# leo27945875/Python_Stable_3D_Truss_Analysis

Measured on AMD Instinct MI355X. Metric: truss solves/sec (batched Solve), higher is better.
Workload: dtype f64; 1 GPU; bar-942_input_0 x 4096 independent copies per GPU (nJ 244, nM 942, n_free 696); batch_per_gpu=4096, parallelism=batch-sharded x1, no collective

## Files before the change

### python_stable_3d_truss_analysis_amd/csrc/order.hip

```cpp
#include "trs_common.h"
#include "../../include/trs_solver.h"
#include <type_traits>

namespace {

#ifndef TRS_ORDER_THREADS
#define TRS_ORDER_THREADS 256
#endif
constexpr int NT = TRS_ORDER_THREADS;
constexpr int NWAVE = NT / 64;
static_assert(NT == 128 || NT == 256 || NT == 512, "two, four or eight waves");
constexpr int ID_BITS = 13;
constexpr int PERMANENT = 0x40000000;
constexpr unsigned long long NO_COST = ~0ull;
constexpr int RCM_BELOW = 128;

struct OrdLds {
    size_t nfr, deg, start, fill, lvl, ppos, queue, nextq, order, ids, frank, bins, adj, adjU, keys,
        cand, best, newidx, c01, cmin, ctrl, red, total;
    int nch_max, n4;
};
__host__ __device__ inline size_t ord_up(size_t v) { return (v + 15) / 16 * 16; }
__host__ __device__ inline OrdLds ord_layout(int nJ_max, int nM_max) {
    OrdLds l;
    const size_t n = (size_t)nJ_max, e = 2 * (size_t)(nM_max < 1 ? 1 : nM_max);
    l.nch_max = 3 * nJ_max / 16 + 8;
    size_t p = 0;
    auto take = [&](size_t bytes) { const size_t at = p; p += ord_up(bytes); return at; };
    l.nfr = take(n);
    l.deg = take(4 * n);
    l.start = take(4 * (n + 1));
    l.fill = take(4 * n);
    l.lvl = take(4 * n);
    l.ppos = take(4 * n);
    l.queue = take(2 * n);
    l.nextq = take(2 * n);
    l.order = take(2 * n);
    l.ids = take(2 * n);
    l.frank = take(2 * (n + 1));
    l.bins = take(2 * 3 * n);
    l.adj = take(2 * (e + 4));
    const size_t shared_at = p;
    l.adjU = take(4 * (e + 4));
    const size_t lists_end = p;
    p = shared_at;
    l.n4 = (nJ_max + 3) / 4 * 4;
    l.keys = take(4 * (size_t)l.n4 * NWAVE);
    l.cand = take(2 * n * NWAVE);
    l.best = take(2 * n * NWAVE);
    l.newidx = take(2 * n * NWAVE);
    l.c01 = take(2 * n * NWAVE);
    p = p > lists_end ? p : lists_end;
    l.cmin = take(4 * (size_t)l.nch_max * NWAVE);
    l.ctrl = take(4 * 32);
    l.red = take(8 * 64);
    l.total = p;
    return l;
}

__device__ __forceinline__ int wave_incl_scan(int v, int lane) {
#pragma unroll
    for (int off = 1; off < 64; off <<= 1) {
        const int up = __shfl_up(v, off);
        if (lane >= off) v += up;
    }
    return v;
}

template <typename T, typename F>
__device__ __forceinline__ T block_reduce(T v, T* red, F op) {
#pragma unroll
    for (int off = 32; off > 0; off >>= 1) v = op(v, __shfl_xor(v, off));
    __syncthreads();
    if ((threadIdx.x & 63) == 0) red[threadIdx.x >> 6] = v;
    __syncthreads();
    T r = red[0];
#pragma unroll
    for (int w = 1; w < NWAVE; ++w) r = op(r, red[w]);
    return r;
}

#ifdef TRS_ORDER_STAMPS
__device__ unsigned long long g_ord_stamps[16];
struct OrdStamp {
    unsigned long long t0;
    __device__ OrdStamp() : t0(__builtin_amdgcn_s_memtime()) {}
    __device__ void mark(int slot) {
        const unsigned long long t = __builtin_amdgcn_s_memtime();
        if ((threadIdx.x & 63) == 0) atomicAdd(&g_ord_stamps[slot], t - t0);
        t0 = t;
    }
};
#else
struct OrdStamp {
    __device__ void mark(int) {}
};
#endif


struct Tables {
    unsigned char* nfr;
    int *deg, *start, *fill, *lvl, *ppos;
    unsigned short *queue, *nextq, *order;
    unsigned short *ids, *frank, *bins, *adj;
    unsigned* adjU;
    unsigned long long* keys;
    unsigned short *cand, *best, *newidx, *c01;
    int *cmin, *ctrl;
    unsigned long long* red;
};

template <bool SORTED>
__device__ int bfs_sweep(const Tables& t, int nj, int root, int stamp, int* last_begin) {
    const int tid = threadIdx.x;
    int* found_cnt = t.ctrl;
    if constexpr (SORTED)
        for (int j = tid; j < nj; j += NT) t.ppos[j] = 0x7fffffff;
    if (tid == 0) {
        t.queue[0] = (unsigned short)root;
        t.lvl[root] = stamp;
        found_cnt[0] = 0;
    }
    __syncthreads();
    unsigned short* found = SORTED ? t.nextq : t.queue;
    int head = 0, tail = 1, depth = 0, begin = 0, turn = 0;
    const int sub = tid & 3;
    while (head < tail) {
        begin = head;
        const int mark = stamp + depth + 1;
        int* my_cnt = found_cnt + turn;
        const int next_turn = turn == 2 ? 0 : turn + 1, slot0 = tail;
        if (tid == 0) found_cnt[next_turn] = 0;
        for (int i = head + (tid >> 2); i < tail; i += NT / 4) {
            const int v = t.queue[i];
            const int e1 = t.start[v + 1];
            for (int e = t.start[v] + sub; e < e1; e += 4) {
                const int w = t.adj[e];
                const int old = atomicMax(&t.lvl[w], mark);
                if (old < stamp) found[slot0 + atomicAdd(my_cnt, 1)] = (unsigned short)w;
                if (SORTED && (old < stamp || old == mark)) atomicMin(&t.ppos[w], i);
            }
        }
        __syncthreads();
        const int new_tail = slot0 + *my_cnt;
        if constexpr (SORTED) {
            const int m = new_tail - tail;
            if (m > 1) {
                for (int x = tid; x < m; x += NT) {
                    const int w = t.nextq[tail + x];
                    t.keys[x] = ((unsigned long long)t.ppos[w] << 40) | ((unsigned long long)t.deg[w] << 20) |
                                (unsigned long long)w;
                }
                __syncthreads();
                for (int x = tid; x < m; x += NT) {
                    const unsigned long long mine = t.keys[x];
                    int rank = 0;
                    for (int y = 0; y < m; ++y) rank += t.keys[y] < mine ? 1 : 0;
                    t.queue[tail + rank] = (unsigned short)(mine & 0xfffffu);
                }
            } else if (m == 1 && tid == 0) {
                t.queue[tail] = t.nextq[tail];
            }
            __syncthreads();
        }
        head = tail;
        tail = new_tail;
        turn = next_turn;
        ++depth;
    }
    *last_begin = begin;
    return tail;
}

template <typename Ord>
__device__ unsigned long long price_order(const Tables& t, int nf, Ord ord, unsigned short* newidx,
                                          unsigned short* c01, int* cmin, int lane, int* n_out) {
    int carry = 0;
    for (int base = 0; base < nf; base += 64) {
        const int k = base + lane;
        const int old = k < nf ? ord(k) : 0;
        const int v = k < nf ? (int)t.nfr[old] : 0;
        const int incl = wave_incl_scan(v, lane);
        const int ds = carry + incl - v;
        if (k < nf) {
            newidx[old] = (unsigned short)k;
            c01[k] = (unsigned short)(((ds >> 4) << 1) | ((((ds + v - 1) >> 4) != (ds >> 4)) ? 1 : 0));
        }
        carry += __shfl(incl, 63);
    }
    const int n = carry, nch = (n + 15) >> 4;
    for (int q = lane; q < nch; q += 64) cmin[q] = q;
    __builtin_amdgcn_wave_barrier();
    for (int k = lane; k < nf; k += 64) {
        const int old = ord(k);
        int m = k;
        const int e1 = t.start[old + 1];
        for (int e = t.start[old]; e < e1; e += 4) {
            const int w0 = t.adj[e], w1 = t.adj[e + 1], w2 = t.adj[e + 2], w3 = t.adj[e + 3];
            const int i0 = newidx[w0], i1 = e + 1 < e1 ? (int)newidx[w1] : k, i2 = e + 2 < e1 ? (int)newidx[w2] : k,
                      i3 = e + 3 < e1 ? (int)newidx[w3] : k;
            m = min(min(m, i0), min(min(i1, i2), i3));
        }
        const int col = c01[m] >> 1, mine = c01[k];
        atomicMin(&cmin[mine >> 1], col);
        if (mine & 1) atomicMin(&cmin[(mine >> 1) + 1], col);
    }
    __builtin_amdgcn_wave_barrier();
    unsigned long long cost = 0;
    int run = nch;
    for (int base = (nch - 1) / 64 * 64; base >= 0; base -= 64) {
        const int q = base + lane;
        int v = q < nch ? cmin[q] : 0x7fffffff;
#pragma unroll
        for (int off = 1; off < 64; off <<= 1) {
            const int o = __shfl_down(v, off);
            if (lane + off < 64) v = min(v, o);
        }
        v = min(v, run);
        if (q < nch) {
            const unsigned long long w = (unsigned long long)(q - v + 1);
            cost += w * (w + 12ull);
        }
        run = __shfl(v, 0);
    }
#pragma unroll
    for (int off = 32; off > 0; off >>= 1) cost += __shfl_xor(cost, off);
    __builtin_amdgcn_wave_barrier();
    *n_out = n;
    return cost;
}

template <typename Fwd>
__device__ void price_order_pair(const Tables& t, int nf, Fwd fwd, unsigned short* newidx, unsigned short* c01,
                                 int* cmin, unsigned short* c01r, int* cminr, int lane, int* n_out,
                                 unsigned long long* cost_fwd, unsigned long long* cost_rev) {
    auto pack = [](int ds, int v) { return (unsigned short)(((ds >> 4) << 1) | ((((ds + v - 1) >> 4) != (ds >> 4)) ? 1 : 0)); };
    int carry = 0;
    for (int base = 0; base < nf; base += 64) {
        const int k = base + lane;
        const int old = k < nf ? fwd(k) : 0;
        const int v = k < nf ? (int)t.nfr[old] : 0;
        const int incl = wave_incl_scan(v, lane);
        const int ds = carry + incl - v;
        if (k < nf) {
            newidx[old] = (unsigned short)k;
            c01[k] = pack(ds, v);
            c01r[k] = (unsigned short)(ds + v);
        }
        carry += __shfl(incl, 63);
    }
    const int n = carry, nch = (n + 15) >> 4;
    for (int q = lane; q < nch; q += 64) {
        cmin[q] = q;
        cminr[q] = q;
    }
    __builtin_amdgcn_wave_barrier();
    for (int k = lane; k < nf; k += 64) {
        const int end = c01r[k];
        c01r[k] = pack(n - end, (int)t.nfr[fwd(k)]);
    }
    __builtin_amdgcn_wave_barrier();
    for (int k = lane; k < nf; k += 64) {
        const int old = fwd(k);
        int lo = k, hi = k;
        const int e1 = t.start[old + 1];
        for (int e = t.start[old]; e < e1; e += 4) {
            const int w0 = t.adj[e], w1 = t.adj[e + 1], w2 = t.adj[e + 2], w3 = t.adj[e + 3];
            const int i0 = newidx[w0], i1 = e + 1 < e1 ? (int)newidx[w1] : k, i2 = e + 2 < e1 ? (int)newidx[w2] : k,
                      i3 = e + 3 < e1 ? (int)newidx[w3] : k;
            lo = min(min(lo, i0), min(min(i1, i2), i3));
            hi = max(max(hi, i0), max(max(i1, i2), i3));
        }
        const int col = c01[lo] >> 1, mine = c01[k];
        atomicMin(&cmin[mine >> 1], col);
        if (mine & 1) atomicMin(&cmin[(mine >> 1) + 1], col);
        const int colr = c01r[hi] >> 1, miner = c01r[k];
        atomicMin(&cminr[miner >> 1], colr);
        if (miner & 1) atomicMin(&cminr[(miner >> 1) + 1], colr);
    }
    __builtin_amdgcn_wave_barrier();
    unsigned long long cf = 0, cr = 0;
    int runf = nch, runr = nch;
    for (int base = (nch - 1) / 64 * 64; base >= 0; base -= 64) {
        const int q = base + lane;
        int vf = q < nch ? cmin[q] : 0x7fffffff, vr = q < nch ? cminr[q] : 0x7fffffff;
#pragma unroll
        for (int off = 1; off < 64; off <<= 1) {
            const int of = __shfl_down(vf, off), orv = __shfl_down(vr, off);
            if (lane + off < 64) {
                vf = min(vf, of);
                vr = min(vr, orv);
            }
        }
        vf = min(vf, runf);
        vr = min(vr, runr);
        if (q < nch) {
            const unsigned long long wf = (unsigned long long)(q - vf + 1), wr = (unsigned long long)(q - vr + 1);
            cf += wf * (wf + 12ull);
            cr += wr * (wr + 12ull);
        }
        runf = __shfl(vf, 0);
        runr = __shfl(vr, 0);
    }
#pragma unroll
    for (int off = 32; off > 0; off >>= 1) {
        cf += __shfl_xor(cf, off);
        cr += __shfl_xor(cr, off);
    }
    __builtin_amdgcn_wave_barrier();
    *n_out = n;
    *cost_fwd = cf;
    *cost_rev = cr;
}

__global__ __launch_bounds__(NT, 4) void trs_joint_order_kernel(
    const double* __restrict__ xyz, const void* __restrict__ conn, const unsigned char* __restrict__ cbits,
    const double* __restrict__ loads, const int* __restrict__ nJ_arr, const int* __restrict__ nM_arr,
    const int nJ_max, const int nM_max, int* __restrict__ perm_out, int* __restrict__ choice_out,
    int* __restrict__ reach_out, double* __restrict__ xyz_out, void* __restrict__ conn_out,
    unsigned char* __restrict__ cbits_out, double* __restrict__ loads_out, const int effort,
    const long long* __restrict__ rows, const int nJ_in, const int nM_in, const double* __restrict__ E_in,
    const double* __restrict__ A_in, double* __restrict__ E_out, double* __restrict__ A_out,
    int* __restrict__ nJ_out, int* __restrict__ nM_out,
    const int conn16, const unsigned char* __restrict__ tidx_in, unsigned char* __restrict__ tidx_out) {
    extern __shared__ unsigned char lds[];
    const int b = blockIdx.x, tid = threadIdx.x, lane = tid & 63;
    const int wave = __builtin_amdgcn_readfirstlane(tid >> 6);
    const size_t src = rows != nullptr ? (size_t)rows[b] : (size_t)b;
    const int nJ_src = rows != nullptr ? nJ_in : nJ_max, nM_src = rows != nullptr ? nM_in : nM_max;
    const int nj = nJ_arr[src], nm = nM_arr[src];
    const OrdLds lay = ord_layout(nJ_max, nM_max);
    Tables t;
    t.nfr = lds + lay.nfr;
    t.deg = reinterpret_cast<int*>(lds + lay.deg);
    t.start = reinterpret_cast<int*>(lds + lay.start);
    t.fill = reinterpret_cast<int*>(lds + lay.fill);
    t.lvl = reinterpret_cast<int*>(lds + lay.lvl);
    t.ppos = reinterpret_cast<int*>(lds + lay.ppos);
    t.queue = reinterpret_cast<unsigned short*>(lds + lay.queue);
    t.nextq = reinterpret_cast<unsigned short*>(lds + lay.nextq);
    t.order = reinterpret_cast<unsigned short*>(lds + lay.order);
    t.ids = reinterpret_cast<unsigned short*>(lds + lay.ids);
    t.frank = reinterpret_cast<unsigned short*>(lds + lay.frank);
    t.bins = reinterpret_cast<unsigned short*>(lds + lay.bins);
    t.adj = reinterpret_cast<unsigned short*>(lds + lay.adj);
    t.adjU = reinterpret_cast<unsigned*>(lds + lay.adjU);
    t.keys = reinterpret_cast<unsigned long long*>(lds + lay.keys);
    t.cand = reinterpret_cast<unsigned short*>(lds + lay.cand);
    t.best = reinterpret_cast<unsigned short*>(lds + lay.best);
    t.newidx = reinterpret_cast<unsigned short*>(lds + lay.newidx);
    t.c01 = reinterpret_cast<unsigned short*>(lds + lay.c01);
    t.cmin = reinterpret_cast<int*>(lds + lay.cmin);
    t.ctrl = reinterpret_cast<int*>(lds + lay.ctrl);
    t.red = reinterpret_cast<unsigned long long*>(lds + lay.red);

    const unsigned char* CB = cbits + src * nJ_src;
    const double* X = xyz + src * 3 * nJ_src;
    int* P = perm_out + (size_t)b * nJ_max;

    OrdStamp st;
    double* Xs = reinterpret_cast<double*>(lds + lay.keys);
    constexpr int MR = 2048 / NT;
    int2 cr[MR];
    const size_t mrow = src * (size_t)nM_src;
    auto CNI = [&](int m) {
        if (conn16) {
            const ushort2 c = reinterpret_cast<const ushort2*>(conn)[mrow + m];
            return int2{(int)c.x, (int)c.y};
        }
        return reinterpret_cast<const int2*>(conn)[mrow + m];
    };
#pragma unroll
    for (int r = 0; r < MR; ++r) {
        const int m = tid + r * NT;
        cr[r] = m < nm ? CNI(m) : int2{0, 0};
    }
    auto for_members = [&](auto&& body) {
#pragma unroll
        for (int r = 0; r < MR; ++r)
            if (tid + r * NT < nm) body(cr[r].x, cr[r].y);
        for (int m = tid + MR * NT; m < nm; m += NT) {
            const int2 c = CNI(m);
            body(c.x, c.y);
        }
    };
    double lo[3] = {X[0], X[1], X[2]}, hi[3] = {X[0], X[1], X[2]};
    for (int j = tid; j < nj; j += NT) {
        const int cb = CB[j];
        t.nfr[j] = (unsigned char)(3 - ((cb & 1) + ((cb >> 1) & 1) + ((cb >> 2) & 1)));
        t.deg[j] = 0;
        t.lvl[j] = 0;
#pragma unroll
        for (int a = 0; a < 3; ++a) {
            const double x = X[3 * j + a];
            Xs[3 * j + a] = x;
            lo[a] = x < lo[a] ? x : lo[a];
            hi[a] = x > hi[a] ? x : hi[a];
        }
    }
    __syncthreads();
    double len2 = 0.0;
    int nlen = 0;
    for_members([&](int a, int c) {
        const double dx = Xs[3 * c] - Xs[3 * a], dy = Xs[3 * c + 1] - Xs[3 * a + 1], dz = Xs[3 * c + 2] - Xs[3 * a + 2];
        const double l2 = dx * dx + dy * dy + dz * dz;
        if (l2 > 0.0) {
            len2 += l2;
            ++nlen;
        }
        if (a == c || t.nfr[a] == 0 || t.nfr[c] == 0) return;
        atomicAdd(&t.deg[a], 1);
        atomicAdd(&t.deg[c], 1);
    });
    __syncthreads();
    if (tid < 64) {
        int base = 0, fbase = 0;
        for (int j0 = 0; j0 < nj; j0 += 64) {
            const int j = j0 + tid;
            const int v = j < nj ? t.deg[j] : 0;
            const int f = j < nj && t.nfr[j] != 0 ? 1 : 0;
            const int incl = wave_incl_scan(v, tid), fincl = wave_incl_scan(f, tid);
            if (j < nj) {
                t.start[j] = base + incl - v;
                t.frank[j] = (unsigned short)(fbase + fincl - f);
                if (f) t.ids[fbase + fincl - f] = (unsigned short)j;
            }
            base += __shfl(incl, 63);
            fbase += __shfl(fincl, 63);
        }
        if (tid == 0) {
            t.start[nj] = base;
            t.frank[nj] = (unsigned short)fbase;
        }
    }
    for (int j = tid; j < nj; j += NT) t.fill[j] = 0;
    __syncthreads();
    const int nf = t.frank[nj];
    {
        double cnt = (double)nlen;
#pragma unroll
        for (int off = 32; off > 0; off >>= 1) {
            len2 += __shfl_xor(len2, off);
            cnt += __shfl_xor(cnt, off);
#pragma unroll
            for (int a = 0; a < 3; ++a) {
                const double l = __shfl_xor(lo[a], off), u = __shfl_xor(hi[a], off);
                lo[a] = l < lo[a] ? l : lo[a];
                hi[a] = u > hi[a] ? u : hi[a];
            }
        }
        double* red = reinterpret_cast<double*>(t.red);
        __syncthreads();
        if (lane == 0) {
            red[8 * wave] = len2;
            red[8 * wave + 1] = cnt;
#pragma unroll
            for (int a = 0; a < 3; ++a) {
                red[8 * wave + 2 + a] = lo[a];
                red[8 * wave + 5 + a] = hi[a];
            }
        }
        __syncthreads();
        len2 = red[0];
        cnt = red[1];
#pragma unroll
        for (int a = 0; a < 3; ++a) {
            lo[a] = red[2 + a];
            hi[a] = red[5 + a];
        }
        for (int w = 1; w < NWAVE; ++w) {
            len2 += red[8 * w];
            cnt += red[8 * w + 1];
#pragma unroll
            for (int a = 0; a < 3; ++a) {
                lo[a] = red[8 * w + 2 + a] < lo[a] ? red[8 * w + 2 + a] : lo[a];
                hi[a] = red[8 * w + 5 + a] > hi[a] ? red[8 * w + 5 + a] : hi[a];
            }
        }
        nlen = (int)cnt;
    }
    const double h = nlen ? (double)(float)(0.25 * sqrt(len2 / (double)nlen)) : 0.0;
    const bool sweeps = h > 0.0 && h < 1e300 && nf > 1 && effort >= 1;
    const bool use_rcm = effort < 3 || nf < RCM_BELOW;
    const int bin_cap = 4 * nJ_max + 64;
    int nb[3] = {1, 1, 1};
    if (sweeps) {
        int top[3] = {1, 1, 1};
        double ha[3];
#pragma unroll
        for (int a = 0; a < 3; ++a) {
            ha[a] = h;
            if (!((hi[a] - lo[a]) / ha[a] < (double)(bin_cap - 2))) ha[a] = (hi[a] - lo[a]) / (double)(bin_cap - 2);
        }
        for (int j = tid; j < nj; j += NT)
#pragma unroll
            for (int a = 0; a < 3; ++a) {
                double q = ha[a] > 0.0 ? (Xs[3 * j + a] - lo[a]) / ha[a] + 0.5 : 0.0;
                if (!(q >= 0.0)) q = 0.0;
                if (q > (double)(bin_cap - 1)) q = (double)(bin_cap - 1);
                t.bins[3 * j + a] = (unsigned short)(int)q;
                top[a] = max(top[a], (int)q + 1);
            }
        int t0 = top[0], t1 = top[1], t2 = top[2];
#pragma unroll
        for (int off = 32; off > 0; off >>= 1) {
            t0 = max(t0, __shfl_xor(t0, off));
            t1 = max(t1, __shfl_xor(t1, off));
            t2 = max(t2, __shfl_xor(t2, off));
        }
        int* redi = reinterpret_cast<int*>(t.red);
        __syncthreads();
        if (lane == 0) {
            redi[4 * wave] = t0;
            redi[4 * wave + 1] = t1;
            redi[4 * wave + 2] = t2;
        }
        __syncthreads();
        for (int w = 0; w < NWAVE; ++w) {
            nb[0] = max(nb[0], redi[4 * w]);
            nb[1] = max(nb[1], redi[4 * w + 1]);
            nb[2] = max(nb[2], redi[4 * w + 2]);
        }
    }
    __syncthreads();
    for_members([&](int a, int c) {
        if (a == c || t.nfr[a] == 0 || t.nfr[c] == 0) return;
        const int ea = t.start[a] + atomicAdd(&t.fill[a], 1), ec = t.start[c] + atomicAdd(&t.fill[c], 1);
        if (use_rcm) {
            t.adjU[ea] = ((unsigned)t.deg[c] << ID_BITS) | (unsigned)c;
            t.adjU[ec] = ((unsigned)t.deg[a] << ID_BITS) | (unsigned)a;
        } else {
            t.adj[ea] = (unsigned short)c;
            t.adj[ec] = (unsigned short)a;
        }
    });
    __syncthreads();
    for (int a = tid >> 2; a < (use_rcm ? nj : 0); a += NT / 4) {
        const int s = t.start[a], d = t.deg[a];
        for (int e = s + (tid & 3); e < s + d; e += 4) {
            const unsigned key = t.adjU[e];
            int rank = 0;
            for (int i = 0; i < d; i += 4) {
                const unsigned k0 = t.adjU[s + i], k1 = t.adjU[s + i + 1], k2 = t.adjU[s + i + 2], k3 = t.adjU[s + i + 3];
                rank += (k0 < key || (k0 == key && s + i < e)) ? 1 : 0;
                rank += (i + 1 < d && (k1 < key || (k1 == key && s + i + 1 < e))) ? 1 : 0;
                rank += (i + 2 < d && (k2 < key || (k2 == key && s + i + 2 < e))) ? 1 : 0;
                rank += (i + 3 < d && (k3 < key || (k3 == key && s + i + 3 < e))) ? 1 : 0;
            }
            t.adj[s + rank] = (unsigned short)(key & ((1u << ID_BITS) - 1));
        }
    }
    __syncthreads();

    st.mark(0);
    int n_order = 0, stamp = 1;
    while (use_rcm) {
        unsigned best = 0xffffffffu;
        for (int j = tid; j < nj; j += NT)
            if (t.nfr[j] != 0 && t.lvl[j] == 0) best = min(best, ((unsigned)t.deg[j] << ID_BITS) | (unsigned)j);
        best = block_reduce(best, reinterpret_cast<unsigned*>(t.red), [](unsigned x, unsigned y) { return min(x, y); });
        if (best == 0xffffffffu) break;
        int root = (int)(best & ((1u << ID_BITS) - 1)), begin = 0, count = 0;
        for (int sweep = 0; sweep < 2; ++sweep) {
            stamp += nj + 2;
            count = bfs_sweep<false>(t, nj, root, stamp, &begin);
            unsigned pick = 0xffffffffu;
            for (int i = begin + tid; i < count; i += NT) {
                const int q = t.queue[i];
                pick = min(pick, ((unsigned)t.deg[q] << ID_BITS) | (unsigned)q);
            }
            pick = block_reduce(pick, reinterpret_cast<unsigned*>(t.red), [](unsigned x, unsigned y) { return min(x, y); });
            root = (int)(pick & ((1u << ID_BITS) - 1));
        }
        stamp += nj + 2;
        count = bfs_sweep<true>(t, nj, root, stamp, &begin);
        __syncthreads();
        for (int i = tid; i < count; i += NT) {
            const int v = t.queue[i];
            t.order[n_order + i] = (unsigned short)v;
            t.lvl[v] = PERMANENT;
        }
        n_order += count;
        __syncthreads();
    }

    st.mark(1);
    __syncthreads();

    st.mark(2);
    auto axis_of = [](int ax, int pos) { return (int)((0x192261624ull >> (6 * ax + 2 * pos)) & 3ull); };
    auto nb_of = [&](int a) { return a == 0 ? nb[0] : (a == 1 ? nb[1] : nb[2]); };
    int first_ax = 0;
    for (int ax = 1; ax < 6; ++ax)
        if (nb_of(axis_of(ax, 0)) > nb_of(axis_of(first_ax, 0)) ||
            (nb_of(axis_of(ax, 0)) == nb_of(axis_of(first_ax, 0)) && nb_of(axis_of(ax, 1)) > nb_of(axis_of(first_ax, 1))))
            first_ax = ax;
#ifndef TRS_ORDER_NSWEEP
#define TRS_ORDER_NSWEEP 6
#endif
    const int n_sweep = sweeps ? (effort >= 2 ? TRS_ORDER_NSWEEP : 1) : 0;
    auto bits_for = [](int count) { int b = 1; while ((1 << b) < count) ++b; return b; };
    const int bits0 = bits_for(nb[0]), bits1 = bits_for(nb[1]), bits2 = bits_for(nb[2]);
    auto bits_of = [&](int a) { return a == 0 ? bits0 : (a == 1 ? bits1 : bits2); };
    const int xbits = bits_for(nf > 1 ? nf : 2);
    const int key_bits = bits0 + bits1 + bits2 + xbits;
    unsigned short* cand = t.cand + (size_t)wave * nJ_max;
    unsigned short* wbest = t.best + (size_t)wave * nJ_max;
    unsigned short* newidx = t.newidx + (size_t)wave * nJ_max;
    unsigned short* c01 = t.c01 + (size_t)wave * nJ_max;
    int* cmin = t.cmin + (size_t)wave * lay.nch_max;
    unsigned* k32 = reinterpret_cast<unsigned*>(t.keys) + (size_t)wave * lay.n4;
    unsigned long long* keys = reinterpret_cast<unsigned long long*>(k32);
    unsigned long long my_cost = NO_COST;
    int my_rank = 0x7fffffff, my_choice = 0, ndof = 0;
    auto consider = [&](unsigned long long cost, int eval_rank, int choice, auto ord) {
        if (cost < my_cost || (cost == my_cost && eval_rank < my_rank)) {
            my_cost = cost;
            my_rank = eval_rank;
            my_choice = choice;
            for (int k = lane; k < nf; k += 64) wbest[k] = (unsigned short)ord(k);
            __builtin_amdgcn_wave_barrier();
        }
    };
    if (nf > 0) {
        if (!use_rcm && !sweeps && wave == 0) {
            auto ord = [&](int k) { return (int)t.ids[k]; };
            consider(price_order(t, nf, ord, newidx, c01, cmin, lane, &ndof), 0, 14, ord);
        }
        if (use_rcm && wave == (n_sweep > 1 ? NWAVE - 2 : 0)) {
            auto ord = [&](int k) { return t.order[nf - 1 - k]; };
            consider(price_order(t, nf, ord, newidx, c01, cmin, lane, &ndof), 0, 0, ord);
        }
        if (use_rcm && wave == (n_sweep > 1 ? NWAVE - 1 : 1)) {
            auto ord = [&](int k) { return t.order[k]; };
            consider(price_order(t, nf, ord, newidx, c01, cmin, lane, &ndof), 1, 1, ord);
        }
        const bool wide_keys = key_bits > 32;
        for (int i = wide_keys ? ((wave & 1) ? n_sweep : wave / 2) : wave; i < n_sweep; i += wide_keys ? NWAVE / 2 : NWAVE) {
#if TRS_ORDER_NSWEEP < 6
            const int ax = i == 0 ? first_ax : (first_ax ^ 1);
#else
            const int ax = i == 0 ? first_ax : (i <= first_ax ? i - 1 : i);
#endif
            const int a0 = axis_of(ax, 0), a1 = axis_of(ax, 1), a2 = axis_of(ax, 2);
            if (!wide_keys) {
                for (int x = lane; x < nf; x += 64) {
                    const int j = t.ids[x];
                    k32[x] = ((((unsigned)t.bins[3 * j + a0] << bits_of(a1) | (unsigned)t.bins[3 * j + a1]) << bits_of(a2) |
                               (unsigned)t.bins[3 * j + a2]) << xbits) | (unsigned)x;
                }
                for (int x = nf + lane; x < ((nf + 3) & ~3); x += 64) k32[x] = 0xffffffffu;
                __builtin_amdgcn_wave_barrier();
                auto rank_pass = [&](auto rc, int x0) {
                    constexpr int R = decltype(rc)::value;
                    unsigned mine[R];
                    int rank[R];
#pragma unroll
                    for (int r = 0; r < R; ++r) {
                        const int x = x0 + lane + 64 * r;
                        mine[r] = x < nf ? k32[x] : 0u;
                        rank[r] = 0;
                    }
#pragma unroll 2
                    for (int y = 0; y < nf; y += 4) {
                        const uint4 kk = *reinterpret_cast<const uint4*>(k32 + y);
#pragma unroll
                        for (int r = 0; r < R; ++r)
                            rank[r] += (kk.x < mine[r] ? 1 : 0) + (kk.y < mine[r] ? 1 : 0) + (kk.z < mine[r] ? 1 : 0) +
                                       (kk.w < mine[r] ? 1 : 0);
                    }
#pragma unroll
                    for (int r = 0; r < R; ++r)
                        if (x0 + lane + 64 * r < nf) cand[rank[r]] = t.ids[mine[r] & ((1u << xbits) - 1)];
                };
                int x0 = 0;
                for (; nf - x0 > 128; x0 += 256) rank_pass(std::integral_constant<int, 4>{}, x0);
                if (nf - x0 > 64) rank_pass(std::integral_constant<int, 2>{}, x0);
                else if (nf - x0 > 0) rank_pass(std::integral_constant<int, 1>{}, x0);
            } else {
                for (int x = lane; x < nf; x += 64) {
                    const int j = t.ids[x];
                    keys[x] = ((unsigned long long)t.bins[3 * j + a0] << (32 + ID_BITS)) |
                              ((unsigned long long)t.bins[3 * j + a1] << (16 + ID_BITS)) |
                              ((unsigned long long)t.bins[3 * j + a2] << ID_BITS) | (unsigned long long)j;
                }
                __builtin_amdgcn_wave_barrier();
                for (int x = lane; x < nf; x += 64) {
                    const unsigned long long mine = keys[x];
                    int rank = 0;
                    int y = 0;
                    for (; y + 1 < nf; y += 2) {
                        const ulonglong2 kk = *reinterpret_cast<const ulonglong2*>(keys + y);
                        rank += (kk.x < mine ? 1 : 0) + (kk.y < mine ? 1 : 0);
                    }
                    if (y < nf) rank += keys[y] < mine ? 1 : 0;
                    cand[rank] = (unsigned short)(mine & ((1ull << ID_BITS) - 1));
                }
            }
            __builtin_amdgcn_wave_barrier();
            st.mark(3);
            auto fwd = [&](int k) { return (int)cand[k]; };
            auto rev = [&](int k) { return (int)cand[nf - 1 - k]; };
            unsigned short* c01r = reinterpret_cast<unsigned short*>(k32);
            int* cminr = reinterpret_cast<int*>(k32 + ((nf + 3) >> 2 << 1));
            unsigned long long cost_fwd, cost_rev;
            price_order_pair(t, nf, fwd, newidx, c01, cmin, c01r, cminr, lane, &ndof, &cost_fwd, &cost_rev);
            consider(cost_fwd, 2 + 2 * i, 2 + 2 * ax, fwd);
            consider(cost_rev, 3 + 2 * i, 3 + 2 * ax, rev);
            st.mark(4);
        }
    }
    st.mark(5);
    if (lane == 0) {
        t.red[wave] = my_cost;
        t.ctrl[8 + wave] = my_rank;
        t.ctrl[16 + wave] = my_choice;
    }
    __syncthreads();
    st.mark(6);
    int win = 0;
    for (int w = 1; w < NWAVE; ++w)
        if (t.red[w] < t.red[win] || (t.red[w] == t.red[win] && t.ctrl[8 + w] < t.ctrl[8 + win])) win = w;
    const unsigned short* wperm = t.best + (size_t)win * nJ_max;
    int* inverse = t.fill;
    int* fullperm = t.ppos;
    for (int k = tid; k < nJ_max; k += NT) {
        if (k < nf) {
            const int old = wperm[k];
            fullperm[k] = old;
            inverse[old] = k;
        } else if (k >= nj) {
            fullperm[k] = k;
        }
    }
    for (int j = tid; j < nj; j += NT)
        if (t.nfr[j] == 0) {
            const int k = nf + j - (int)t.frank[j];
            fullperm[k] = j;
            inverse[j] = k;
        }
    if (tid == 0 && choice_out != nullptr) choice_out[b] = nf > 0 ? t.ctrl[16 + win] : 0;
    __syncthreads();
    for (int k = tid; k < nJ_max; k += NT) P[k] = fullperm[k];
    if (reach_out != nullptr && wave == 0) {
        int widest = 0;
        if (nf > 0) {
            auto ord = [&](int k) { return (int)wperm[k]; };
            int n = 0;
            price_order(t, nf, ord, newidx, c01, cmin, lane, &n);
            const int nch = (n + 15) >> 4, nchp = (n + 63) / 64 * 4;
            int* ft = cmin;
            for (int q = nch + lane; q < nchp; q += 64) ft[q] = q;
            __builtin_amdgcn_wave_barrier();
            int run = nchp;
            for (int base = (nchp - 1) / 64 * 64; base >= 0; base -= 64) {
                const int q = base + lane;
                int v = q < nchp ? ft[q] : 0x7fffffff;
#pragma unroll
                for (int off = 1; off < 64; off <<= 1) {
                    const int o = __shfl_down(v, off);
                    if (lane + off < 64) v = min(v, o);
                }
                v = min(v, run);
                if (q < nchp) ft[q] = v;
                run = __shfl(v, 0);
            }
            __builtin_amdgcn_wave_barrier();
            for (int j = lane; j < nchp / 4; j += 64) {
                const int tcol = 4 * j + 3;
                int q = tcol;
                while (q + 1 < nchp && ft[q + 1] <= tcol) ++q;
                widest = max(widest, q - tcol);
            }
#pragma unroll
            for (int off = 32; off > 0; off >>= 1) widest = max(widest, __shfl_xor(widest, off));
        }
        if (lane == 0) reach_out[b] = widest;
    }
    st.mark(7);
    if (xyz_out != nullptr) {
        const double* F = loads + src * 3 * nJ_src;
        double* XO = xyz_out + (size_t)b * 3 * nJ_max;
        double* FO = loads_out + (size_t)b * 3 * nJ_max;
        unsigned char* CO = cbits_out + (size_t)b * nJ_max;
        for (int j = tid; j < nJ_max; j += NT) {
            const int k = j < nj ? inverse[j] : j;
            const bool in = rows == nullptr || j < nj;
            const double x0 = in ? X[3 * j] : 0.0, x1 = in ? X[3 * j + 1] : 0.0, x2 = in ? X[3 * j + 2] : 0.0;
            const double f0 = in ? F[3 * j] : 0.0, f1 = in ? F[3 * j + 1] : 0.0, f2 = in ? F[3 * j + 2] : 0.0;
            const unsigned char cb = in ? CB[j] : (unsigned char)0;
            XO[3 * k] = x0; XO[3 * k + 1] = x1; XO[3 * k + 2] = x2;
            FO[3 * k] = f0; FO[3 * k + 1] = f1; FO[3 * k + 2] = f2;
            CO[k] = cb;
        }
        for (int m = tid; m < nM_max; m += NT) {
            int2 c = {0, 0};
            if (m < nm) {
                c = CNI(m);
                c.x = inverse[c.x];
                c.y = inverse[c.y];
            }
            if (conn16) reinterpret_cast<ushort2*>(conn_out)[(size_t)b * nM_max + m] = ushort2{(unsigned short)c.x, (unsigned short)c.y};
            else reinterpret_cast<int2*>(conn_out)[(size_t)b * nM_max + m] = c;
        }
    }
    if (rows != nullptr) {
        if (tidx_in != nullptr) {
            const unsigned char* TI = tidx_in + src * nM_src;
            unsigned char* TO = tidx_out + (size_t)b * nM_max;
            for (int m = tid; m < nM_max; m += NT) TO[m] = m < nm ? TI[m] : (unsigned char)0;
        } else {
            const double* EI = E_in + src * nM_src;
            const double* AI = A_in + src * nM_src;
            double* EO = E_out + (size_t)b * nM_max;
            double* AO = A_out + (size_t)b * nM_max;
            for (int m = tid; m < nM_max; m += NT) {
                EO[m] = m < nm ? EI[m] : 0.0;
                AO[m] = m < nm ? AI[m] : 0.0;
            }
        }
        if (tid == 0) {
            nJ_out[b] = nj;
            nM_out[b] = nm;
        }
    }
    st.mark(8);
}

}


#ifdef TRS_ORDER_STAMPS
extern "C" int trs_order_debug_stamps(unsigned long long* host_out, int reset) {
    int rc = (int)hipMemcpyFromSymbol(host_out, HIP_SYMBOL(g_ord_stamps), sizeof(g_ord_stamps));
    if (reset) {
        unsigned long long zero[16] = {0};
        rc |= (int)hipMemcpyToSymbol(HIP_SYMBOL(g_ord_stamps), zero, sizeof(zero));
    }
    return rc;
}
#endif

extern "C" int trs_joint_order_fits(int nJ_max, int nM_max) {
    if (nJ_max <= 0 || nM_max < 0 || nJ_max >= (1 << ID_BITS) || nM_max >= 65536) return 0;
    return ord_layout(nJ_max, nM_max).total <= 160 * 1024 ? 1 : 0;
}

extern "C" int trs_joint_order_launch(int B, int nJ_max, int nM_max, const double* xyz, const void* conn,
                                      const unsigned char* cbits, const double* loads, const int* nJ, const int* nM,
                                      int* perm, int* choice, int* reach, double* xyz_out, void* conn_out,
                                      unsigned char* cbits_out, double* loads_out, int effort, hipStream_t stream,
                                      const long long* rows, int nJ_in, int nM_in, const double* E_in,
                                      const double* A_in, double* E_out, double* A_out, int* nJ_out, int* nM_out,
                                      int conn16, const unsigned char* tidx_in, unsigned char* tidx_out) {
    if (B <= 0) return 0;
    if (!trs_joint_order_fits(nJ_max, nM_max)) return (int)hipErrorInvalidValue;
    const size_t lds = ord_layout(nJ_max, nM_max).total
        ;
    if (lds > 64 * 1024) {
        static const int raised = (int)hipFuncSetAttribute(reinterpret_cast<const void*>(trs_joint_order_kernel),
                                                           hipFuncAttributeMaxDynamicSharedMemorySize, 160 * 1024);
        (void)raised;
    }
    hipLaunchKernelGGL(trs_joint_order_kernel, dim3(B), dim3(NT), lds, stream, xyz, conn, cbits, loads, nJ, nM, nJ_max,
                       nM_max, perm, choice, reach, xyz_out, conn_out, cbits_out, loads_out, effort, rows, nJ_in, nM_in,
                       E_in, A_in, E_out, A_out, nJ_out, nM_out, conn16, tidx_in, tidx_out);
    return (int)hipGetLastError();
}
```

Measured before the change: 2.692 million solves/s.

## Fold reach computation into order pricing and raise order kernel occupancy

Each candidate ordering's pricing pass now also computes a per-lane reach term from the suffix-min chunk profile. The winning candidate's reach is recorded alongside its cost, so the final re-pricing and separate reach scan on wave 0 after selection are removed. The launch-bounds minimum workgroups per CU goes from 4 to 6, and the per-thread register array size is made configurable. The closed-form reach term must match the old padded scan exactly, and tighter launch bounds may cause register spills.

Measured after the change: 2.743 million solves/s, median of 6. 1.02x the previous value.

```diff
diff --git a/python_stable_3d_truss_analysis_amd/csrc/order.hip b/python_stable_3d_truss_analysis_amd/csrc/order.hip
--- a/python_stable_3d_truss_analysis_amd/csrc/order.hip
+++ b/python_stable_3d_truss_analysis_amd/csrc/order.hip
@@ -6,6 +6,12 @@
 
 #ifndef TRS_ORDER_THREADS
 #define TRS_ORDER_THREADS 256
+#endif
+#ifndef TRS_ORDER_MIN_WG
+#define TRS_ORDER_MIN_WG 6
+#endif
+#ifndef TRS_ORDER_MR
+#define TRS_ORDER_MR (2048 / TRS_ORDER_THREADS)
 #endif
 constexpr int NT = TRS_ORDER_THREADS;
 constexpr int NWAVE = NT / 64;
@@ -172,9 +178,11 @@
     return tail;
 }
 
+__device__ __forceinline__ int reach_term(int q, int ft) { return q - (ft & ~3) - 3; }
+
 template <typename Ord>
 __device__ unsigned long long price_order(const Tables& t, int nf, Ord ord, unsigned short* newidx,
-                                          unsigned short* c01, int* cmin, int lane, int* n_out) {
+                                          unsigned short* c01, int* cmin, int lane, int* n_out, int* reach_lane) {
     int carry = 0;
     for (int base = 0; base < nf; base += 64) {
         const int k = base + lane;
@@ -207,7 +215,7 @@
     }
     __builtin_amdgcn_wave_barrier();
     unsigned long long cost = 0;
-    int run = nch;
+    int run = nch, reach = 0;
     for (int base = (nch - 1) / 64 * 64; base >= 0; base -= 64) {
         const int q = base + lane;
         int v = q < nch ? cmin[q] : 0x7fffffff;
@@ -220,6 +228,7 @@
         if (q < nch) {
             const unsigned long long w = (unsigned long long)(q - v + 1);
             cost += w * (w + 12ull);
+            reach = max(reach, reach_term(q, v));
         }
         run = __shfl(v, 0);
     }
@@ -227,13 +236,15 @@
     for (int off = 32; off > 0; off >>= 1) cost += __shfl_xor(cost, off);
     __builtin_amdgcn_wave_barrier();
     *n_out = n;
+    *reach_lane = reach;
     return cost;
 }
 
 template <typename Fwd>
 __device__ void price_order_pair(const Tables& t, int nf, Fwd fwd, unsigned short* newidx, unsigned short* c01,
                                  int* cmin, unsigned short* c01r, int* cminr, int lane, int* n_out,
-                                 unsigned long long* cost_fwd, unsigned long long* cost_rev) {
+                                 unsigned long long* cost_fwd, unsigned long long* cost_rev, int* reach_fwd,
+                                 int* reach_rev) {
     auto pack = [](int ds, int v) { return (unsigned short)(((ds >> 4) << 1) | ((((ds + v - 1) >> 4) != (ds >> 4)) ? 1 : 0)); };
     int carry = 0;
     for (int base = 0; base < nf; base += 64) {
@@ -280,7 +291,7 @@
     }
     __builtin_amdgcn_wave_barrier();
     unsigned long long cf = 0, cr = 0;
-    int runf = nch, runr = nch;
+    int runf = nch, runr = nch, rf = 0, rr = 0;
     for (int base = (nch - 1) / 64 * 64; base >= 0; base -= 64) {
         const int q = base + lane;
         int vf = q < nch ? cmin[q] : 0x7fffffff, vr = q < nch ? cminr[q] : 0x7fffffff;
@@ -298,6 +309,8 @@
             const unsigned long long wf = (unsigned long long)(q - vf + 1), wr = (unsigned long long)(q - vr + 1);
             cf += wf * (wf + 12ull);
             cr += wr * (wr + 12ull);
+            rf = max(rf, reach_term(q, vf));
+            rr = max(rr, reach_term(q, vr));
         }
         runf = __shfl(vf, 0);
         runr = __shfl(vr, 0);
@@ -311,9 +324,11 @@
     *n_out = n;
     *cost_fwd = cf;
     *cost_rev = cr;
-}
-
-__global__ __launch_bounds__(NT, 4) void trs_joint_order_kernel(
+    *reach_fwd = rf;
+    *reach_rev = rr;
+}
+
+__global__ __launch_bounds__(NT, TRS_ORDER_MIN_WG) void trs_joint_order_kernel(
     const double* __restrict__ xyz, const void* __restrict__ conn, const unsigned char* __restrict__ cbits,
     const double* __restrict__ loads, const int* __restrict__ nJ_arr, const int* __restrict__ nM_arr,
     const int nJ_max, const int nM_max, int* __restrict__ perm_out, int* __restrict__ choice_out,
@@ -360,7 +375,7 @@
 
     OrdStamp st;
     double* Xs = reinterpret_cast<double*>(lds + lay.keys);
-    constexpr int MR = 2048 / NT;
+    constexpr int MR = TRS_ORDER_MR;
     int2 cr[MR];
     const size_t mrow = src * (size_t)nM_src;
     auto CNI = [&](int m) {
@@ -612,12 +627,15 @@
     unsigned* k32 = reinterpret_cast<unsigned*>(t.keys) + (size_t)wave * lay.n4;
     unsigned long long* keys = reinterpret_cast<unsigned long long*>(k32);
     unsigned long long my_cost = NO_COST;
-    int my_rank = 0x7fffffff, my_choice = 0, ndof = 0;
-    auto consider = [&](unsigned long long cost, int eval_rank, int choice, auto ord) {
+    int my_rank = 0x7fffffff, my_choice = 0, my_reach = 0, ndof = 0, rl = 0;
+    auto consider = [&](unsigned long long cost, int eval_rank, int choice, auto ord, int reach_lane) {
         if (cost < my_cost || (cost == my_cost && eval_rank < my_rank)) {
             my_cost = cost;
             my_rank = eval_rank;
             my_choice = choice;
+#pragma unroll
+            for (int off = 32; off > 0; off >>= 1) reach_lane = max(reach_lane, __shfl_xor(reach_lane, off));
+            my_reach = __builtin_amdgcn_readfirstlane(reach_lane);
             for (int k = lane; k < nf; k += 64) wbest[k] = (unsigned short)ord(k);
             __builtin_amdgcn_wave_barrier();
         }
@@ -625,15 +643,18 @@
     if (nf > 0) {
         if (!use_rcm && !sweeps && wave == 0) {
             auto ord = [&](int k) { return (int)t.ids[k]; };
-            consider(price_order(t, nf, ord, newidx, c01, cmin, lane, &ndof), 0, 14, ord);
+            const unsigned long long cost = price_order(t, nf, ord, newidx, c01, cmin, lane, &ndof, &rl);
+            consider(cost, 0, 14, ord, rl);
         }
         if (use_rcm && wave == (n_sweep > 1 ? NWAVE - 2 : 0)) {
             auto ord = [&](int k) { return t.order[nf - 1 - k]; };
-            consider(price_order(t, nf, ord, newidx, c01, cmin, lane, &ndof), 0, 0, ord);
+            const unsigned long long cost = price_order(t, nf, ord, newidx, c01, cmin, lane, &ndof, &rl);
+            consider(cost, 0, 0, ord, rl);
         }
         if (use_rcm && wave == (n_sweep > 1 ? NWAVE - 1 : 1)) {
             auto ord = [&](int k) { return t.order[k]; };
-            consider(price_order(t, nf, ord, newidx, c01, cmin, lane, &ndof), 1, 1, ord);
+            const unsigned long long cost = price_order(t, nf, ord, newidx, c01, cmin, lane, &ndof, &rl);
+            consider(cost, 1, 1, ord, rl);
         }
         const bool wide_keys = key_bits > 32;
         for (int i = wide_keys ? ((wave & 1) ? n_sweep : wave / 2) : wave; i < n_sweep; i += wide_keys ? NWAVE / 2 : NWAVE) {
@@ -704,9 +725,10 @@
             unsigned short* c01r = reinterpret_cast<unsigned short*>(k32);
             int* cminr = reinterpret_cast<int*>(k32 + ((nf + 3) >> 2 << 1));
             unsigned long long cost_fwd, cost_rev;
-            price_order_pair(t, nf, fwd, newidx, c01, cmin, c01r, cminr, lane, &ndof, &cost_fwd, &cost_rev);
-            consider(cost_fwd, 2 + 2 * i, 2 + 2 * ax, fwd);
-            consider(cost_rev, 3 + 2 * i, 3 + 2 * ax, rev);
+            int rl_rev = 0;
+            price_order_pair(t, nf, fwd, newidx, c01, cmin, c01r, cminr, lane, &ndof, &cost_fwd, &cost_rev, &rl, &rl_rev);
+            consider(cost_fwd, 2 + 2 * i, 2 + 2 * ax, fwd, rl);
+            consider(cost_rev, 3 + 2 * i, 3 + 2 * ax, rev, rl_rev);
             st.mark(4);
         }
     }
@@ -715,6 +737,7 @@
         t.red[wave] = my_cost;
         t.ctrl[8 + wave] = my_rank;
         t.ctrl[16 + wave] = my_choice;
+        t.ctrl[24 + wave] = my_reach;
     }
     __syncthreads();
     st.mark(6);
@@ -742,41 +765,7 @@
     if (tid == 0 && choice_out != nullptr) choice_out[b] = nf > 0 ? t.ctrl[16 + win] : 0;
     __syncthreads();
     for (int k = tid; k < nJ_max; k += NT) P[k] = fullperm[k];
-    if (reach_out != nullptr && wave == 0) {
-        int widest = 0;
-        if (nf > 0) {
-            auto ord = [&](int k) { return (int)wperm[k]; };
-            int n = 0;
-            price_order(t, nf, ord, newidx, c01, cmin, lane, &n);
-            const int nch = (n + 15) >> 4, nchp = (n + 63) / 64 * 4;
-            int* ft = cmin;
-            for (int q = nch + lane; q < nchp; q += 64) ft[q] = q;
-            __builtin_amdgcn_wave_barrier();
-            int run = nchp;
-            for (int base = (nchp - 1) / 64 * 64; base >= 0; base -= 64) {
-                const int q = base + lane;
-                int v = q < nchp ? ft[q] : 0x7fffffff;
-#pragma unroll
-                for (int off = 1; off < 64; off <<= 1) {
-                    const int o = __shfl_down(v, off);
-                    if (lane + off < 64) v = min(v, o);
-                }
-                v = min(v, run);
-                if (q < nchp) ft[q] = v;
-                run = __shfl(v, 0);
-            }
-            __builtin_amdgcn_wave_barrier();
-            for (int j = lane; j < nchp / 4; j += 64) {
-                const int tcol = 4 * j + 3;
-                int q = tcol;
-                while (q + 1 < nchp && ft[q + 1] <= tcol) ++q;
-                widest = max(widest, q - tcol);
-            }
-#pragma unroll
-            for (int off = 32; off > 0; off >>= 1) widest = max(widest, __shfl_xor(widest, off));
-        }
-        if (lane == 0) reach_out[b] = widest;
-    }
+    if (reach_out != nullptr && tid == 0) reach_out[b] = nf > 0 ? t.ctrl[24 + win] : 0;
     st.mark(7);
     if (xyz_out != nullptr) {
         const double* F = loads + src * 3 * nJ_src;
```
